# limanling/clip-event

Hardware: AMD Instinct MI355X
Metric: image-text pairs/sec/GPU, ViT-B/32 224px x 77-tok, global-batch contrastive (higher is better)
Workload: dtype bf16; 1 GPU; ViT-B/32 224px x 77-tok, bf16 operands, per-GPU batch 256, K=1, InfoNCE only, full train step (fwd+bwd+clip_grad_norm+Adam), random-init weights; global_batch=256, parallelism=dp1, captions=SOT + U[8,75] random ids + EOT, zero-padded to 77 (SURVEY 8(d) c2), text_rows=live tokens SOT..EOT only: 54.8% of B*77 rows (identical results, see DESIGN.md), fresh_captions_every_step=True, alignment=False, cu_hog=0, nt_pgrid=256, full=False

## Files before the change

clip_event_amd/csrc/attention.hip:

```cpp
#include <map>
#include <mutex>

#include <type_traits>

#include "common.hpp"
#include "../../include/clip_event_hip.h"

namespace {

constexpr int HD = 64;
constexpr int ROW = 160;

typedef __attribute__((address_space(3))) s16x4 lds_s16x4;
typedef __attribute__((ext_vector_type(8))) short s16x8;

__device__ __forceinline__ bf16x8 tr_pair(const char* p0, const char* p1) {
    s16x4 lo = __builtin_amdgcn_ds_read_tr16_b64_v4i16((lds_s16x4*)p0);
    s16x4 hi = __builtin_amdgcn_ds_read_tr16_b64_v4i16((lds_s16x4*)p1);
    s16x8 v = {lo[0], lo[1], lo[2], lo[3], hi[0], hi[1], hi[2], hi[3]};
    return __builtin_bit_cast(bf16x8, v);
}

__device__ __forceinline__ bf16x8 pack8(const f32x4& a, const f32x4& b) {
    u32x4 v = {pack_bf2(a[0], a[1]), pack_bf2(a[2], a[3]), pack_bf2(b[0], b[1]), pack_bf2(b[2], b[3])};
// ... 11 lines not shown
        const int idx = tid + j * nthr, r = idx >> 3, c = idx & 7;
        const uint32_t off = r < L ? (uint32_t)(r * ld * 2 + c * 16) : 0x80000000u;
        kv[j] = __builtin_amdgcn_raw_buffer_load_b128(rK, off, 0, 0);
        vv[j] = __builtin_amdgcn_raw_buffer_load_b128(rV, off, 0, 0);
    }
#pragma unroll
    for (int j = 0; j < NCH; ++j) {
        const int idx = tid + j * nthr, r = idx >> 3, c = idx & 7;
        if (idx < Lp * 8) {
            *reinterpret_cast<u32x4*>(sK + r * ROW + c * 16) = kv[j];
            *reinterpret_cast<u32x4*>(sV + r * ROW + c * 16) = vv[j];
        }
    }
}

template <int T>
__global__ __launch_bounds__(512) void attn_fwd_kernel(const bf16_t* __restrict__ qkv, long ld, bf16_t* __restrict__ o,
                                                       long ldo, float* __restrict__ lse,
                                                       const int* __restrict__ cu, int Lmax, int H, int D,
                                                       int causal, float scale) {
    extern __shared__ __attribute__((aligned(16))) char smem[];
    constexpr int Lp = T * 16;
    char* sK = smem;
    char* sV = smem + Lp * ROW;
    const int tid = threadIdx.x, lane = tid & 63;
    const int wave = __builtin_amdgcn_readfirstlane(tid >> 6), nw = blockDim.x >> 6;
    const int b = blockIdx.x / H, h = blockIdx.x - b * H;
    const long row0 = cu ? (long)cu[b] : (long)b * Lmax;
    const int L = cu ? min(cu[b + 1] - cu[b], Lmax) : Lmax;
    if (L <= 0) return;
    const int Tl = ((L + 31) >> 5) << 1;
    const bf16_t* base = qkv + row0 * ld + h * HD;

    const int li = lane & 15, g = lane >> 4;
    const int nstrips = (L + 15) >> 4;
    const int strip = wave;
    const int i = strip * 16 + li;
    const int iq = min(i, L - 1);
    bf16x8 qf[2];
    if (strip < nstrips) {
#pragma unroll
        for (int ks = 0; ks < 2; ++ks)
            qf[ks] = *reinterpret_cast<const bf16x8*>(base + (long)iq * ld + ks * 32 + g * 8);
    }
    stage_kv<4>(sK, sV, base + D, base + 2 * D, ld, L, Tl * 16, tid, blockDim.x);
    __syncthreads();

    if (strip < nstrips) {
        f32x4 s[T];
#pragma unroll
        for (int t = 0; t < T; ++t) {
            s[t] = f32x4{0.f, 0.f, 0.f, 0.f};
            if (t < Tl) {
#pragma unroll
                for (int ks = 0; ks < 2; ++ks) {
                    bf16x8 kf = *reinterpret_cast<const bf16x8*>(sK + (t * 16 + li) * ROW + (ks * 4 + g) * 16);
                    s[t] = __builtin_amdgcn_mfma_f32_16x16x32_bf16(kf, qf[ks], s[t], 0, 0, 0);
                }
            }
        }
        float mx = -INFINITY;
#pragma unroll
        for (int t = 0; t < T; ++t)
#pragma unroll
            for (int r = 0; r < 4; ++r) {
                const int j = t * 16 + g * 4 + r;
                const bool ok = (j < L) && (!causal || j <= i);
                s[t][r] = ok ? s[t][r] * scale : -INFINITY;
                mx = fmaxf(mx, s[t][r]);
            }
        mx = fmaxf(mx, __shfl_xor(mx, 16, 64));
        mx = fmaxf(mx, __shfl_xor(mx, 32, 64));
        float sum = 0.f;
#pragma unroll
        for (int t = 0; t < T; ++t)
#pragma unroll
            for (int r = 0; r < 4; ++r) {
                s[t][r] = __expf(s[t][r] - mx);
                sum += s[t][r];
            }
        sum += __shfl_xor(sum, 16, 64);
        sum += __shfl_xor(sum, 32, 64);
        f32x4 acc[4];
#pragma unroll
        for (int ct = 0; ct < 4; ++ct) acc[ct] = f32x4{0.f, 0.f, 0.f, 0.f};
#pragma unroll
        for (int sidx = 0; sidx < T / 2; ++sidx) {
            if (2 * sidx >= Tl) continue;
            bf16x8 pf = pack8(s[2 * sidx], s[2 * sidx + 1]);
            const char* vrow = sV + (32 * sidx + 4 * g + (li >> 2)) * ROW + (4 * (li & 3)) * 2;
#pragma unroll
            for (int ct = 0; ct < 4; ++ct) {
                bf16x8 vf = tr_pair(vrow + ct * 32, vrow + ct * 32 + 16 * ROW);
                acc[ct] = __builtin_amdgcn_mfma_f32_16x16x32_bf16(vf, pf, acc[ct], 0, 0, 0);
            }
        }
        if (i < L) {
            const float inv = 1.0f / sum;
            bf16_t* orow = o + (row0 + i) * ldo + h * HD + 4 * g;
#pragma unroll
            for (int ct = 0; ct < 4; ++ct) {
                u32x2 pk = {pack_bf2(acc[ct][0] * inv, acc[ct][1] * inv), pack_bf2(acc[ct][2] * inv, acc[ct][3] * inv)};
                *reinterpret_cast<u32x2*>(orow + ct * 16) = pk;
            }
            if (g == 0) lse[((long)b * H + h) * Lmax + i] = mx + __logf(sum);
        }
    }
}

template <int T>
__global__ __launch_bounds__(512) void attn_bwd_kernel(const bf16_t* __restrict__ qkv, long ld,
                                                       const bf16_t* __restrict__ o, long ldo,
                                                       const bf16_t* __restrict__ dout, long lddo,
                                                       const float* __restrict__ lse, bf16_t* __restrict__ dqkv,
                                                       long lddq, float* __restrict__ bias_grad,
                                                       const int* __restrict__ cu, int Lmax, int H, int D,
                                                       int causal, float scale) {
    extern __shared__ __attribute__((aligned(16))) char smem[];
    constexpr int Lp = T * 16;
    constexpr int PROW = Lp * 2 + 32;
    char* sA = smem;
    char* sB = sA + Lp * ROW;
    char* sP = sB + Lp * ROW;
    char* sDS = sP + Lp * PROW;
    auto csum = [&](int i) __attribute__((always_inline)) -> float* { return reinterpret_cast<float*>(sP + (i >> 3) * PROW + Lp * 2 + (i & 7) * 4); };
    const int tid = threadIdx.x, lane = tid & 63;
    const int wave = __builtin_amdgcn_readfirstlane(tid >> 6), nw = blockDim.x >> 6;
    const int b = blockIdx.x / H, h = blockIdx.x - b * H;
    const long row0 = cu ? (long)cu[b] : (long)b * Lmax;
    const int L = cu ? min(cu[b + 1] - cu[b], Lmax) : Lmax;
    if (L <= 0) return;
    const int Tl = ((L + 31) >> 5) << 1;
    const int Ll = Tl * 16;
    const bf16_t* base = qkv + row0 * ld + h * HD;
    const bf16_t* dob = dout + row0 * lddo + h * HD;
    const bf16_t* ob = o + row0 * ldo + h * HD;
    bf16_t* dbase = dqkv + row0 * lddq + h * HD;

    for (int i = tid; i < 192; i += blockDim.x) *csum(i) = 0.f;
    const int li = lane & 15, g = lane >> 4;
    u32x4 rK[2], rV[2], rQ[2], rD[2];
#pragma unroll
    for (int c = 0; c < 2; ++c) {
        const int idx = tid + c * blockDim.x;
        const int r = idx >> 3, ch = idx & 7;
        const u32x4 z = {0u, 0u, 0u, 0u};
        rK[c] = z; rV[c] = z; rQ[c] = z; rD[c] = z;
        if (idx < Ll * 8 && r < L) {
            rK[c] = *reinterpret_cast<const u32x4*>(base + D + (long)r * ld + ch * 8);
            rV[c] = *reinterpret_cast<const u32x4*>(base + 2 * D + (long)r * ld + ch * 8);
            rQ[c] = *reinterpret_cast<const u32x4*>(base + (long)r * ld + ch * 8);
            rD[c] = *reinterpret_cast<const u32x4*>(dob + (long)r * lddo + ch * 8);
        }
    }
    const int strip = wave;
    const bool has_strip = strip < Tl;
    const int i = strip * 16 + li;
    const bool iok = has_strip && i < L;
    const int iq = min(i, L - 1);
    float dl = 0.f, lsei = 0.f;
    bf16x8 qf[2], df[2];
    if (has_strip) {
        const u32x4* pd = reinterpret_cast<const u32x4*>(dob + (long)iq * lddo + g * 16);
        const u32x4* po = reinterpret_cast<const u32x4*>(ob + (long)iq * ldo + g * 16);
#pragma unroll
        for (int v = 0; v < 2; ++v) {
            u32x4 a = pd[v], c = po[v];
#pragma unroll
            for (int e = 0; e < 4; ++e) dl += bf_lo(a[e]) * bf_lo(c[e]) + bf_hi(a[e]) * bf_hi(c[e]);
        }
        lsei = lse[((long)b * H + h) * Lmax + iq];
#pragma unroll
        for (int ks = 0; ks < 2; ++ks) {
            qf[ks] = *reinterpret_cast<const bf16x8*>(base + (long)iq * ld + ks * 32 + g * 8);
            df[ks] = *reinterpret_cast<const bf16x8*>(dob + (long)iq * lddo + ks * 32 + g * 8);
        }
    }
#pragma unroll
    for (int c = 0; c < 2; ++c) {
        const int idx = tid + c * blockDim.x;
        if (idx < Ll * 8) {
            *reinterpret_cast<u32x4*>(sA + (idx >> 3) * ROW + (idx & 7) * 16) = rK[c];
            *reinterpret_cast<u32x4*>(sB + (idx >> 3) * ROW + (idx & 7) * 16) = rV[c];
        }
    }
    __syncthreads();
    dl += __shfl_xor(dl, 16, 64);
    dl += __shfl_xor(dl, 32, 64);

    if (has_strip) {
        f32x4 p[T], ds[T];
#pragma unroll
        for (int t = 0; t < T; ++t) {
            p[t] = f32x4{0.f, 0.f, 0.f, 0.f};
            ds[t] = f32x4{0.f, 0.f, 0.f, 0.f};
            if (t >= Tl) continue;
#pragma unroll
            for (int ks = 0; ks < 2; ++ks) {
                bf16x8 kf = *reinterpret_cast<const bf16x8*>(sA + (t * 16 + li) * ROW + (ks * 4 + g) * 16);
                bf16x8 vf = *reinterpret_cast<const bf16x8*>(sB + (t * 16 + li) * ROW + (ks * 4 + g) * 16);
                p[t] = __builtin_amdgcn_mfma_f32_16x16x32_bf16(kf, qf[ks], p[t], 0, 0, 0);
                ds[t] = __builtin_amdgcn_mfma_f32_16x16x32_bf16(vf, df[ks], ds[t], 0, 0, 0);
            }
#pragma unroll
            for (int r = 0; r < 4; ++r) {
                const int j = t * 16 + g * 4 + r;
                const bool ok = iok && (j < L) && (!causal || j <= i);
                const float pv = ok ? __expf(p[t][r] * scale - lsei) : 0.f;
                p[t][r] = pv;
                ds[t][r] = pv * (ds[t][r] - dl) * scale;
            }
            u32x2 pk = {pack_bf2(p[t][0], p[t][1]), pack_bf2(p[t][2], p[t][3])};
            u32x2 dk = {pack_bf2(ds[t][0], ds[t][1]), pack_bf2(ds[t][2], ds[t][3])};
            *reinterpret_cast<u32x2*>(sP + i * PROW + (t * 16 + g * 4) * 2) = pk;
            *reinterpret_cast<u32x2*>(sDS + i * PROW + (t * 16 + g * 4) * 2) = dk;
        }
        f32x4 acc[4];
#pragma unroll
        for (int ct = 0; ct < 4; ++ct) acc[ct] = f32x4{0.f, 0.f, 0.f, 0.f};
#pragma unroll
        for (int sidx = 0; sidx < T / 2; ++sidx) {
            if (2 * sidx >= Tl) continue;
            bf16x8 sf = pack8(ds[2 * sidx], ds[2 * sidx + 1]);
            const char* krow = sA + (32 * sidx + 4 * g + (li >> 2)) * ROW + (4 * (li & 3)) * 2;
#pragma unroll
            for (int ct = 0; ct < 4; ++ct) {
                bf16x8 kf = tr_pair(krow + ct * 32, krow + ct * 32 + 16 * ROW);
                acc[ct] = __builtin_amdgcn_mfma_f32_16x16x32_bf16(kf, sf, acc[ct], 0, 0, 0);
            }
        }
        if (iok) {
            bf16_t* qrow = dbase + (long)i * lddq + 4 * g;
#pragma unroll
            for (int ct = 0; ct < 4; ++ct) {
                u32x2 pk = {pack_bf2(acc[ct][0], acc[ct][1]), pack_bf2(acc[ct][2], acc[ct][3])};
                *reinterpret_cast<u32x2*>(qrow + ct * 16) = pk;
            }
// ... 19 lines not shown
        }
    }
    __syncthreads();
    const int nkt = (L + 15) >> 4;
    for (int jt = wave; jt < nkt; jt += nw) {
        const int j = jt * 16 + li;
        f32x4 av[4], ak[4];
#pragma unroll
        for (int ct = 0; ct < 4; ++ct) {
            av[ct] = f32x4{0.f, 0.f, 0.f, 0.f};
            ak[ct] = f32x4{0.f, 0.f, 0.f, 0.f};
        }
#pragma unroll
        for (int sidx = 0; sidx < T / 2; ++sidx) {
            if (2 * sidx >= Tl) continue;
            const int irow = 32 * sidx + 8 * g + (li >> 2);
            const char* pcol = sP + irow * PROW + (jt * 16 + 4 * (li & 3)) * 2;
            const char* scol = sDS + irow * PROW + (jt * 16 + 4 * (li & 3)) * 2;
            bf16x8 pf = tr_pair(pcol, pcol + 4 * PROW);
            bf16x8 sf = tr_pair(scol, scol + 4 * PROW);
            const int roff = irow * ROW + (4 * (li & 3)) * 2;
#pragma unroll
            for (int ct = 0; ct < 4; ++ct) {
                bf16x8 dof = tr_pair(sB + roff + ct * 32, sB + roff + ct * 32 + 4 * ROW);
                bf16x8 qf = tr_pair(sA + roff + ct * 32, sA + roff + ct * 32 + 4 * ROW);
                av[ct] = __builtin_amdgcn_mfma_f32_16x16x32_bf16(dof, pf, av[ct], 0, 0, 0);
                ak[ct] = __builtin_amdgcn_mfma_f32_16x16x32_bf16(qf, sf, ak[ct], 0, 0, 0);
            }
        }
        if (j < L) {
// ... 546 lines not shown
    }
    return e.p;
}

}

#define ATTN_DISPATCH(T, CALL)                 \
    switch (T) {                               \
        case 2: CALL(2); break;                \
        case 4: CALL(4); break;                \
        case 6: CALL(6); break;                \
        case 8: CALL(8); break;                \
        default: CE_CHECK_ARG(false, "attention: sequence length %d not supported", L); \
    }

extern "C" int ce_attention_fwd(const void* qkv, long ld, void* o, long ldo, float* lse, const int* cu_seqlens, int B,
                                int L, int H, int causal, void* stream) {
    CE_CHECK_ARG(B > 0 && L > 0 && H > 0, "ce_attention_fwd: empty problem");
    CE_CHECK_ARG(ld % 8 == 0 && ldo % 4 == 0, "ce_attention_fwd: ld must be a multiple of 8, ldo of 4");
    const int D = H * HD;
    if (L > 128) {
        CE_CHECK_ARG(!cu_seqlens, "ce_attention_fwd: packed batches are limited to 128 tokens per sample");
        CE_CHECK_ARG((long)B * H <= 65535, "ce_attention_fwd: B*H = %ld exceeds the grid", (long)B * H);
        hipStream_t sl = (hipStream_t)stream;
        CeProfScope prof(CE_PROF_ATTN_FWD, 4.0 * B * H * (double)L * L * HD, 2.0 * (double)B * L * (4.0 * D), sl);
        static const int ns = getenv("CE_ATTN_NS_FWD") ? atoi(getenv("CE_ATTN_NS_FWD")) : 1;
        if (ns == 1)
            hipLaunchKernelGGL(attn_fwd_long_kernel<1>, dim3((L + LB - 1) / LB, B * H), dim3(256), 0, sl, (const bf16_t*)qkv, ld,
                               (bf16_t*)o, ldo, lse, L, H, D, causal, 0.125f, attn_xcd_order());
        else
            hipLaunchKernelGGL(attn_fwd_long_kernel<2>, dim3((L + 2 * LB - 1) / (2 * LB), B * H), dim3(256), 0, sl, (const bf16_t*)qkv, ld,
                               (bf16_t*)o, ldo, lse, L, H, D, causal, 0.125f, attn_xcd_order());
        CE_LAUNCH_CHECK();
        return 0;
    }
    const int T = tiles_for(L);
    const int Lp = T * 16;
    int nw = (L + 15) / 16;
    if (nw > 8) nw = 8;
    const size_t lds = 2 * (size_t)Lp * ROW;
    const float scale = 0.125f;
    hipStream_t s = (hipStream_t)stream;
    CeProfScope prof(CE_PROF_ATTN_FWD, 4.0 * B * H * (double)L * L * HD, 2.0 * (double)B * L * (4.0 * D), s);
#define CALL(TT)                                                                                              \
    hipLaunchKernelGGL(attn_fwd_kernel<TT>, dim3(B * H), dim3(64 * nw), lds, s, (const bf16_t*)qkv, ld, (bf16_t*)o, ldo, \
                       lse, cu_seqlens, L, H, D, causal, scale)
    ATTN_DISPATCH(T, CALL);
#undef CALL
    CE_LAUNCH_CHECK();
    return 0;
}

extern "C" int ce_attention_bwd(const void* qkv, long ld, const void* o, long ldo, const void* dout, long lddo,
                                const float* lse, void* dqkv, long lddq, float* bias_grad, const int* cu_seqlens, int B,
                                int L, int H, int causal, void* stream) {
    CE_CHECK_ARG(B > 0 && L > 0 && H > 0, "ce_attention_bwd: empty problem");
    CE_CHECK_ARG(ld % 8 == 0 && ldo % 8 == 0 && lddo % 8 == 0 && lddq % 4 == 0, "ce_attention_bwd: bad leading dimension");
    const int D = H * HD;
    if (L > 128) {
        CE_CHECK_ARG(!cu_seqlens, "ce_attention_bwd: packed batches are limited to 128 tokens per sample");
        CE_CHECK_ARG((long)B * H <= 65535, "ce_attention_bwd: B*H = %ld exceeds the grid", (long)B * H);
        hipStream_t sl = (hipStream_t)stream;
        CeProfScope prof(CE_PROF_ATTN_BWD, 14.0 * B * H * (double)L * L * HD, 2.0 * (double)B * L * (8.0 * D), sl);
        static const int ns = getenv("CE_ATTN_NS") ? atoi(getenv("CE_ATTN_NS")) : 2;
        static const int nk = getenv("CE_ATTN_NK") ? atoi(getenv("CE_ATTN_NK")) : 1;
// ... 6 lines not shown
        if (ns == 1)
            hipLaunchKernelGGL(attn_bwd_long_dq_kernel<1>, grid1, dim3(256), 0, sl, (const bf16_t*)qkv, ld, (const bf16_t*)o, ldo,
                               (const bf16_t*)dout, lddo, lse, (bf16_t*)dqkv, lddq, bias_grad, delta, L, H, D, causal, 0.125f, attn_xcd_order());
        else
            hipLaunchKernelGGL(attn_bwd_long_dq_kernel<2>, grid2, dim3(256), 0, sl, (const bf16_t*)qkv, ld, (const bf16_t*)o, ldo,
                               (const bf16_t*)dout, lddo, lse, (bf16_t*)dqkv, lddq, bias_grad, delta, L, H, D, causal, 0.125f, attn_xcd_order());
        if (nk == 1)
            hipLaunchKernelGGL(attn_bwd_long_dkv_kernel<1>, grid1, dim3(256), 0, sl, (const bf16_t*)qkv, ld, (const bf16_t*)o, ldo,
                               (const bf16_t*)dout, lddo, lse, (bf16_t*)dqkv, lddq, bias_grad, delta, L, H, D, causal, 0.125f, attn_xcd_order());
        else
            hipLaunchKernelGGL(attn_bwd_long_dkv_kernel<2>, grid2, dim3(256), 0, sl, (const bf16_t*)qkv, ld, (const bf16_t*)o, ldo,
                               (const bf16_t*)dout, lddo, lse, (bf16_t*)dqkv, lddq, bias_grad, delta, L, H, D, causal, 0.125f, attn_xcd_order());
        CE_LAUNCH_CHECK();
        return 0;
    }
    const int T = tiles_for(L);
    const int Lp = T * 16;
    int nw = T;
    if (nw > 8) nw = 8;
    const size_t lds = 2 * (size_t)Lp * ROW + 2 * (size_t)Lp * (Lp * 2 + 32);
    const float scale = 0.125f;
    hipStream_t s = (hipStream_t)stream;
    CeProfScope prof(CE_PROF_ATTN_BWD, 10.0 * B * H * (double)L * L * HD, 2.0 * (double)B * L * (8.0 * D), s);
#define CALL(TT)                                                                                                   \
    do {                                                                                                           \
        static std::once_flag attr;                                                                                \
        std::call_once(attr, [] {                                                                                  \
            hipFuncSetAttribute(reinterpret_cast<const void*>(attn_bwd_kernel<TT>),                                \
                                hipFuncAttributeMaxDynamicSharedMemorySize, 160 * 1024);                           \
        });                                                                                                        \
        hipLaunchKernelGGL(attn_bwd_kernel<TT>, dim3(B * H), dim3(64 * nw), lds, s, (const bf16_t*)qkv, ld,        \
                           (const bf16_t*)o, ldo, (const bf16_t*)dout, lddo, lse, (bf16_t*)dqkv, lddq, bias_grad, cu_seqlens, L, \
                           H, D, causal, scale);                                                                           \
    } while (0)
    ATTN_DISPATCH(T, CALL);
#undef CALL
    CE_LAUNCH_CHECK();
    return 0;
}
```

clip_event_amd/csrc/tower.cpp:

```cpp
#include <hip/hip_runtime.h>
#include <stdlib.h>

#include <map>
#include <mutex>

#include "common.hpp"
#include "../../include/clip_event_hip.h"

namespace {

constexpr int WG_MAX_BLOCKS = 8;
constexpr int WG_SETS = WG_MAX_BLOCKS + 1;
constexpr int LNP_RING = 8;

struct Carver {
    char* base;
    size_t off = 0;
    explicit Carver(void* b) : base(reinterpret_cast<char*>(b)) {}
    template <typename T>
    T* take(size_t n) {
        off = (off + 255) & ~size_t(255);
        T* p = base ? reinterpret_cast<T*>(base + off) : nullptr;
        off += n * sizeof(T);
        return p;
// ... 113 lines not shown
        if (rc__ != 0) return rc__; \
    } while (0)

int linear(bool use8, const Layout& L, const void*& q8_of, const void* A, long lda, const void* W, const void* W8, const float* S8, int M,
           int N, int K, int epi, const float* bias, const void* resid, long ldr, void* out, long ldo, void* out2,
           long ldo2, const void* aux, long ldaux, void* stream) {
    if (use8 && W8 && S8 && K % 128 == 0 && K <= 4096) {
        if (q8_of != A || lda != K) TRY(ce_quant_rows_fp8(A, lda, L.q8, K, L.q8s, M, K, stream));
        q8_of = nullptr;
        return ce_gemm_nt_fp8(L.q8, K, L.q8s, W8, K, S8, M, N, K, epi, bias, resid, ldr, out, ldo, out2, ldo2, aux, ldaux,
                              stream);
    }
    return ce_gemm_nt(A, lda, W, K, M, N, K, epi, bias, resid, ldr, out, ldo, out2, ldo2, aux, ldaux, stream);
}

int forward_run(const ce_tower_desc* d, int batch, int rows, const int* cu_seqlens, const void* x0, Layout& L, void* x_out,
                const int* sel_rows, bool infer, void* stream) {
    const int M = rows, w = d->width;
    const bool f8 = (d->fp8 & 1) != 0;
    const int ST = d->stream16 ? CE_T_F16 : CE_T_F32;
    const int EPI_RESID = d->stream16 ? CE_EPI_BIAS_RESID_F16 : CE_EPI_BIAS_RESID_F32;
    const int EPI_FC = infer ? CE_EPI_BIAS_QGELU_BF16 : CE_EPI_BIAS_GELU;
    const long esz = d->stream16 ? 2 : 4;
    const void* x = x0;
    const void* q8_of = nullptr;
    const bool lnq = f8 && w % 128 == 0 && w <= 4096;
    for (int l = 0; l < d->layers; ++l) {
        const ce_block_params& p = d->blocks[l];
        BlockStash& s = L.blk[l];
        void* xo = (l + 1 < d->layers) ? s.x_out : x_out;
        TRY(ce_layernorm_fwd_q8(x, ST, w, nullptr, p.ln1_w, p.ln1_b, s.h1, CE_T_BF16, w, s.mean1, s.rstd1, M, w, 1e-5f,
                                lnq ? L.q8 : nullptr, w, L.q8s, stream));
        if (lnq) q8_of = s.h1;
        TRY(linear(f8, L, q8_of, s.h1, w, p.w_qkv, p.w8_qkv, p.s8_qkv, M, 3 * w, w, CE_EPI_BIAS_BF16, p.b_qkv, nullptr, 0, s.qkv, 3 * w, nullptr, 0,
                       nullptr, 0, stream));
        TRY(ce_attention_fwd(s.qkv, 3 * w, s.o, w, s.lse, cu_seqlens, batch, d->tokens, d->heads, d->causal, stream));
        if (sel_rows && l + 1 == d->layers) {
            const int Bn = batch;
            TRY(ce_copy_rows(s.o, w * 2L, sel_rows, L.os, w * 2L, nullptr, Bn, w * 2, stream));
            TRY(ce_copy_rows(x, w * esz, sel_rows, L.xs_in, w * esz, nullptr, Bn, (int)(w * esz), stream));
            TRY(linear(f8, L, q8_of, L.os, w, p.w_out, p.w8_out, p.s8_out, Bn, w, w, EPI_RESID, p.b_out, L.xs_in, w, L.xs_mid, w, nullptr,
                           0, nullptr, 0, stream));
            TRY(ce_layernorm_fwd_t(L.xs_mid, ST, w, nullptr, p.ln2_w, p.ln2_b, L.h2s, CE_T_BF16, w, L.means, L.rstds, Bn, w, 1e-5f, stream));
            TRY(linear(f8, L, q8_of, L.h2s, w, p.w_fc, p.w8_fc, p.s8_fc, Bn, 4 * w, w, EPI_FC, p.b_fc, nullptr, 0, infer ? L.gs : L.as, 4 * w,
                           infer ? nullptr : L.gs, infer ? 0 : 4 * w, nullptr, 0, stream));
            TRY(linear(f8, L, q8_of, L.gs, 4 * w, p.w_proj, p.w8_proj, p.s8_proj, Bn, w, 4 * w, EPI_RESID, p.b_proj, L.xs_mid, w, x_out, w,
                           nullptr, 0, nullptr, 0, stream));
            break;
        }
        TRY(linear(f8, L, q8_of, s.o, w, p.w_out, p.w8_out, p.s8_out, M, w, w, EPI_RESID, p.b_out, x, w, s.x_mid, w, nullptr, 0, nullptr,
                       0, stream));
        TRY(ce_layernorm_fwd_q8(s.x_mid, ST, w, nullptr, p.ln2_w, p.ln2_b, s.h2, CE_T_BF16, w, s.mean2, s.rstd2, M, w, 1e-5f,
                                lnq ? L.q8 : nullptr, w, L.q8s, stream));
        if (lnq) q8_of = s.h2;
// ... 140 lines not shown
        const int l = top, Bn = batch, q = l % WG_SETS;
        const ce_block_params& p = d->blocks[l];
        BlockStash& s = L.blk[l];
        const void* x_in = (l == 0) ? x0 : L.blk[l - 1].x_out;
        TRY(ce_cast_bf16(dx_sel, L.dxbs, (long)Bn * w, stream));
        TRY(linear(b8, L, q8_of, L.dxbs, w, p.wt_proj, p.wt8_proj, p.st8_proj, Bn, 4 * w, w, CE_EPI_GELUGRAD_BF16, nullptr, nullptr, 0, L.das, 4 * w, nullptr,
                       0, L.as, 4 * w, stream));
        TRY(ce_colsum_bf16(L.dxbs, w, p.g_b_proj, Bn, w, stream));
        TRY(linear(b8, L, q8_of, L.das, 4 * w, p.wt_fc, p.wt8_fc, p.st8_fc, Bn, w, 4 * w, CE_EPI_BF16, nullptr, nullptr, 0, L.dhs, w, nullptr, 0,
                       nullptr, 0, stream));
        TRY(ce_colsum_bf16(L.das, 4 * w, p.g_b_fc, Bn, 4 * w, stream));
        TRY(ce_layernorm_bwd_t(L.dhs, CE_T_BF16, w, L.xs_mid, ST, w, nullptr, L.means, L.rstds, p.ln2_w, dx_sel, CE_T_F32, L.dxs_mid,
                               ST, w, L.dxb2s, w, p.g_ln2_w, p.g_ln2_b, p.g_b_out, GS, Bn, w, stream));
        TRY(linear(b8, L, q8_of, L.dxb2s, w, p.wt_out, p.wt8_out, p.st8_out, Bn, w, w, CE_EPI_BF16, nullptr, nullptr, 0, L.dos, w, nullptr, 0, nullptr, 0,
                       stream));
        TRY(ce_scatter_rows_zero(L.dos, w * 2L, L.d_o, w * 2L, sel_rows, Bn, M, w * 2, stream));
        TRY(ce_attention_bwd(s.qkv, 3 * w, s.o, w, L.d_o, w, s.lse, L.dqkv[q], 3 * w, p.g_b_qkv, cu_seqlens, batch, d->tokens, d->heads,
                             d->causal, stream));
        {
            const void* P[3] = {L.dxbs, L.das, L.dxb2s};
            const long ldp[3] = {w, 4L * w, w};
            const void* Q[3] = {L.gs, L.h2s, L.os};
            const long ldq[3] = {4L * w, w, w};
            const int Nn[3] = {w, 4 * w, w};
            const int Kk[3] = {4 * w, w, w};
            float* out[3] = {p.g_w_proj, p.g_w_fc, p.g_w_out};
            const long ldo[3] = {4L * w, w, w};
            TRY(ce_gemm_tn_grouped_ex(3, P, ldp, Q, ldq, Bn, Nn, Kk, out, ldo, 0, d->wgrad_overwrite, stream));
        }
        queue(L.dqkv[q], 3L * w, s.h1, w, 3 * w, w, p.g_w_qkv, w);
        TRY(linear(b8, L, q8_of, L.dqkv[q], 3 * w, p.wt_qkv, p.wt8_qkv, p.st8_qkv, M, w, 3 * w, CE_EPI_BF16, nullptr, nullptr, 0, L.dh, w, nullptr, 0,
                       nullptr, 0, stream));
        TRY(ce_scatter_rows_zero(L.dxs_mid, w * esz, dx, w * esz, sel_rows, Bn, M, (int)(w * esz), stream));
// ... 45 lines not shown
```

clip_event_amd/ops.py:

```python
from __future__ import annotations

from ctypes import c_float, c_int, c_long, c_void_p
from typing import Optional

import torch

from . import _lib as L
from ._lib import check, lib, ptr, stream


def _rows(t: torch.Tensor) -> int:
    return t.shape[0]


def gemm_nt(a: torch.Tensor, b: torch.Tensor, epilogue: int, *, bias=None, resid=None, out=None, out2=None,
            aux=None, M: Optional[int] = None) -> torch.Tensor:
    assert a.dtype == torch.bfloat16 and b.dtype == torch.bfloat16 and a.is_cuda and b.is_cuda
    M = a.shape[0] if M is None else M
    K = a.shape[1]
    N = b.shape[0]
    assert b.shape[1] == K
    f32_out = epilogue in (L.EPI_F32, L.EPI_BIAS_F32, L.EPI_BIAS_RESID_F32)
    if epilogue == L.EPI_BIAS_RESID_F16:
        assert resid is not None and resid.dtype == torch.float16
# ... 89 lines not shown
    check(lib().ce_cast_t(ptr(x), c_int(_TYPE[x.dtype]), ptr(y), c_int(_TYPE[dtype]), c_float(mul), c_long(x.numel()), stream()),
          "ce_cast_t")
    return y


def attention_fwd(qkv: torch.Tensor, B: int, L: int, H: int, causal: bool, cu_seqlens=None):
    assert qkv.dtype == torch.bfloat16
    o = torch.empty(qkv.shape[0], H * 64, device=qkv.device, dtype=torch.bfloat16)
    lse = torch.empty(B * H * L, device=qkv.device, dtype=torch.float32)
    check(lib().ce_attention_fwd(ptr(qkv), c_long(qkv.stride(0)), ptr(o), c_long(o.stride(0)), ptr(lse),
                                 ptr(cu_seqlens), c_int(B), c_int(L), c_int(H), c_int(1 if causal else 0), stream()),
          "ce_attention_fwd")
    return o, lse


def attention_bwd(qkv, o, dout, lse, B: int, L: int, H: int, causal: bool, bias_grad=None, cu_seqlens=None):
    dqkv = torch.empty_like(qkv)
    check(lib().ce_attention_bwd(ptr(qkv), c_long(qkv.stride(0)), ptr(o), c_long(o.stride(0)), ptr(dout),
                                 c_long(dout.stride(0)), ptr(lse), ptr(dqkv), c_long(dqkv.stride(0)), ptr(bias_grad),
                                 ptr(cu_seqlens), c_int(B), c_int(L), c_int(H), c_int(1 if causal else 0), stream()),
          "ce_attention_bwd")
    return dqkv


def probe_mfma(shape: int, a_frags: torch.Tensor, b_frags: torch.Tensor) -> torch.Tensor:
    out = torch.empty(64, 4 if shape == 16 else 16, device=a_frags.device, dtype=torch.float32)
    check(lib().ce_probe_mfma(c_int(shape), ptr(a_frags), ptr(b_frags), ptr(out), stream()), "ce_probe_mfma")
    return out


def probe_tr16(image: torch.Tensor, byte_off: torch.Tensor) -> torch.Tensor:
    out = torch.empty(64, 4, device=image.device, dtype=torch.int16)
    check(lib().ce_probe_tr16(ptr(image), c_int(image.numel()), ptr(byte_off), ptr(out), stream()), "ce_probe_tr16")
    return out


# ... 70 lines not shown
```

include/clip_event_hip.h:

```cpp
#ifndef CLIP_EVENT_HIP_H
#define CLIP_EVENT_HIP_H

#include <stddef.h>
#include <stdint.h>

#ifdef __cplusplus
extern "C" {
#endif

const char* ce_last_error(void);
int ce_version(void);

enum {
    CE_EPI_BF16 = 0,
    CE_EPI_F32 = 1,
    CE_EPI_BIAS_BF16 = 2,
    CE_EPI_BIAS_F32 = 3,
    CE_EPI_BIAS_RESID_F32 = 4,
    CE_EPI_BIAS_GELU = 5,
    CE_EPI_GELUGRAD_BF16 = 6,
    CE_EPI_BIAS_RESID_F16 = 7,
    CE_EPI_BIAS_QGELU_BF16 = 8
};

// ... 64 lines not shown
                              const float* gscale, int M, int D, void* q8, long ldq, float* qscale, float* partials,
                              void* stream);
#define CE_LN_FOLD_MAX 64
typedef struct ce_ln_fold_job {
    const float* partials;
    float *dw, *db, *dxsum;
    int blocks, D;
} ce_ln_fold_job;
int ce_layernorm_fold(const ce_ln_fold_job* jobs , int njobs, void* stream);

int ce_attention_fwd(const void* qkv, long ld, void* o, long ldo, float* lse, const int* cu_seqlens, int B, int L,
                     int H, int causal, void* stream);
int ce_attention_bwd(const void* qkv, long ld, const void* o, long ldo, const void* dout, long lddo,
                     const float* lse, void* dqkv, long lddq, float* bias_grad, const int* cu_seqlens, int B, int L,
                     int H, int causal, void* stream);

int ce_im2col(const float* image, void* patches, int B, int resolution, int patch, int k_padded, void* stream);
int ce_vision_assemble(const float* patch_out, const float* cls, const float* pos, float* x0, int B, int tokens,
                       int D, void* stream);
int ce_vision_assemble_bwd(const float* dx0, void* dpatch, int B, int tokens, int D, void* stream);
int ce_token_embed(const int64_t* ids, const int* src_rows, const float* table, const float* pos, float* x0, long rows,
                   int tokens, int D, int vocab, void* stream);
int ce_token_embed_t(const int64_t* ids, const int* src_rows, const float* table, const float* pos, void* x0, int x0_type,
                     long rows, int tokens, int D, int vocab, void* stream);
int ce_token_embed_bwd(const int64_t* ids, const int* src_rows, const float* dx0, float* dtable, long rows, int D,
                       int vocab, void* stream);
int ce_pos_embed_bwd_packed(const float* dx0, const int* cu_seqlens, float* dpos, int n, int tokens, int D,
                            void* stream);
int ce_batch_reduce(const float* x, float* out, int B, long slab, long n, int accumulate, void* stream);
int ce_colsum_bf16(const void* x, long ld, float* out, int M, int N, void* stream);
// ... 173 lines not shown
```

Before: 20270 pairs/s (whole job).

## Add selected-row attention for last layer, causal tile skipping, and length-class launches

In the final transformer layer only the selected output row per sample (e.g. CLS/EOT) is needed. New fwd/bwd 'rows' kernels therefore compute attention only for that query strip, and the separate copy_rows and scatter_rows_zero passes are dropped. The kernels also gain compile-time causal and rows flags. With causal masking they skip key tiles above the diagonal using a per-strip unrolled dispatch. Packed variable-length batches are launched as several length classes so short sequences use smaller tile counts. This adds more template instantiations and launches, plus extra zeroing logic in the backward pass for strips that are not selected.

```diff
diff --git a/clip_event_amd/csrc/attention.hip b/clip_event_amd/csrc/attention.hip
--- a/clip_event_amd/csrc/attention.hip
+++ b/clip_event_amd/csrc/attention.hip
@@ -49,13 +49,27 @@
     }
 }
 
-template <int T>
+template <int N, class F>
+__device__ __forceinline__ void dispatch_upto(int v, F& f) {
+    if constexpr (N >= 1) {
+        if (v == N) f(std::integral_constant<int, N>{});
+        else dispatch_upto<N - 1>(v, f);
+    }
+}
+
+template <int T, bool CAUSAL, bool ROWS>
 __global__ __launch_bounds__(512) void attn_fwd_kernel(const bf16_t* __restrict__ qkv, long ld, bf16_t* __restrict__ o,
                                                        long ldo, float* __restrict__ lse,
-                                                       const int* __restrict__ cu, int Lmax, int H, int D,
-                                                       int causal, float scale) {
+                                                       const int* __restrict__ cu, const int* __restrict__ sel, int Lmax, int tl_min,
+                                                       int H, int D, float scale) {
     extern __shared__ __attribute__((aligned(16))) char smem[];
     constexpr int Lp = T * 16;
+    constexpr bool causal = CAUSAL;
+#ifdef CE_DIAG_NO_CAUSAL_SKIP
+    constexpr bool SKIP = false;
+#else
+    constexpr bool SKIP = CAUSAL;
+#endif
     char* sK = smem;
     char* sV = smem + Lp * ROW;
     const int tid = threadIdx.x, lane = tid & 63;
@@ -65,6 +79,7 @@
     const int L = cu ? min(cu[b + 1] - cu[b], Lmax) : Lmax;
     if (L <= 0) return;
     const int Tl = ((L + 31) >> 5) << 1;
+    if (Tl <= tl_min || Tl > T) return;
     const bf16_t* base = qkv + row0 * ld + h * HD;
 
     const int li = lane & 15, g = lane >> 4;
@@ -72,8 +87,14 @@
     const int strip = wave;
     const int i = strip * 16 + li;
     const int iq = min(i, L - 1);
+    int isel = 0;
+    if constexpr (ROWS) {
+        isel = (int)((long)sel[b] - row0);
+        if (isel < 0 || isel >= L) return;
+    }
+    const bool active = ROWS ? strip == (isel >> 4) : strip < nstrips;
     bf16x8 qf[2];
-    if (strip < nstrips) {
+    if (active) {
 #pragma unroll
         for (int ks = 0; ks < 2; ++ks)
             qf[ks] = *reinterpret_cast<const bf16x8*>(base + (long)iq * ld + ks * 32 + g * 8);
@@ -81,12 +102,14 @@
     stage_kv<4>(sK, sV, base + D, base + 2 * D, ld, L, Tl * 16, tid, blockDim.x);
     __syncthreads();
 
-    if (strip < nstrips) {
-        f32x4 s[T];
-#pragma unroll
-        for (int t = 0; t < T; ++t) {
+    auto strip_body = [&](auto te_tag) __attribute__((always_inline)) {
+        constexpr int TE = decltype(te_tag)::value;
+        constexpr int TP = TE + (TE & 1);
+        f32x4 s[TP];
+#pragma unroll
+        for (int t = 0; t < TP; ++t) {
             s[t] = f32x4{0.f, 0.f, 0.f, 0.f};
-            if (t < Tl) {
+            if (t < TE && (SKIP || t < Tl)) {
 #pragma unroll
                 for (int ks = 0; ks < 2; ++ks) {
                     bf16x8 kf = *reinterpret_cast<const bf16x8*>(sK + (t * 16 + li) * ROW + (ks * 4 + g) * 16);
@@ -96,7 +119,7 @@
         }
         float mx = -INFINITY;
 #pragma unroll
-        for (int t = 0; t < T; ++t)
+        for (int t = 0; t < TE; ++t)
 #pragma unroll
             for (int r = 0; r < 4; ++r) {
                 const int j = t * 16 + g * 4 + r;
@@ -108,7 +131,7 @@
         mx = fmaxf(mx, __shfl_xor(mx, 32, 64));
         float sum = 0.f;
 #pragma unroll
-        for (int t = 0; t < T; ++t)
+        for (int t = 0; t < TE; ++t)
 #pragma unroll
             for (int r = 0; r < 4; ++r) {
                 s[t][r] = __expf(s[t][r] - mx);
@@ -120,8 +143,8 @@
 #pragma unroll
         for (int ct = 0; ct < 4; ++ct) acc[ct] = f32x4{0.f, 0.f, 0.f, 0.f};
 #pragma unroll
-        for (int sidx = 0; sidx < T / 2; ++sidx) {
-            if (2 * sidx >= Tl) continue;
+        for (int sidx = 0; sidx < (TE + 1) / 2; ++sidx) {
+            if (!SKIP && 2 * sidx >= Tl) continue;
             bf16x8 pf = pack8(s[2 * sidx], s[2 * sidx + 1]);
             const char* vrow = sV + (32 * sidx + 4 * g + (li >> 2)) * ROW + (4 * (li & 3)) * 2;
 #pragma unroll
@@ -130,9 +153,9 @@
                 acc[ct] = __builtin_amdgcn_mfma_f32_16x16x32_bf16(vf, pf, acc[ct], 0, 0, 0);
             }
         }
-        if (i < L) {
+        if (ROWS ? i == isel : i < L) {
             const float inv = 1.0f / sum;
-            bf16_t* orow = o + (row0 + i) * ldo + h * HD + 4 * g;
+            bf16_t* orow = o + (ROWS ? (long)b : row0 + i) * ldo + h * HD + 4 * g;
 #pragma unroll
             for (int ct = 0; ct < 4; ++ct) {
                 u32x2 pk = {pack_bf2(acc[ct][0] * inv, acc[ct][1] * inv), pack_bf2(acc[ct][2] * inv, acc[ct][3] * inv)};
@@ -140,19 +163,29 @@
             }
             if (g == 0) lse[((long)b * H + h) * Lmax + i] = mx + __logf(sum);
         }
-    }
-}
-
-template <int T>
+    };
+    if (active) {
+        if constexpr (SKIP) dispatch_upto<T>(strip + 1, strip_body);
+        else strip_body(std::integral_constant<int, T>{});
+    }
+}
+
+template <int T, bool CAUSAL, bool ROWS>
 __global__ __launch_bounds__(512) void attn_bwd_kernel(const bf16_t* __restrict__ qkv, long ld,
                                                        const bf16_t* __restrict__ o, long ldo,
                                                        const bf16_t* __restrict__ dout, long lddo,
                                                        const float* __restrict__ lse, bf16_t* __restrict__ dqkv,
                                                        long lddq, float* __restrict__ bias_grad,
-                                                       const int* __restrict__ cu, int Lmax, int H, int D,
-                                                       int causal, float scale) {
+                                                       const int* __restrict__ cu, const int* __restrict__ sel, int Lmax, int tl_min,
+                                                       int H, int D, float scale) {
     extern __shared__ __attribute__((aligned(16))) char smem[];
     constexpr int Lp = T * 16;
+    constexpr bool causal = CAUSAL;
+#ifdef CE_DIAG_NO_CAUSAL_SKIP
+    constexpr bool SKIP = false;
+#else
+    constexpr bool SKIP = CAUSAL;
+#endif
     constexpr int PROW = Lp * 2 + 32;
     char* sA = smem;
     char* sB = sA + Lp * ROW;
@@ -166,11 +199,18 @@
     const int L = cu ? min(cu[b + 1] - cu[b], Lmax) : Lmax;
     if (L <= 0) return;
     const int Tl = ((L + 31) >> 5) << 1;
+    if (Tl <= tl_min || Tl > T) return;
     const int Ll = Tl * 16;
     const bf16_t* base = qkv + row0 * ld + h * HD;
-    const bf16_t* dob = dout + row0 * lddo + h * HD;
-    const bf16_t* ob = o + row0 * ldo + h * HD;
+    const bf16_t* dob = dout + (ROWS ? (long)b : row0) * lddo + h * HD;
+    const bf16_t* ob = o + (ROWS ? (long)b : row0) * ldo + h * HD;
     bf16_t* dbase = dqkv + row0 * lddq + h * HD;
+    int isel = -1;
+    if constexpr (ROWS) {
+        isel = (int)((long)sel[b] - row0);
+        if (isel < 0 || isel >= L) isel = -1;
+    }
+    const int ssel = isel >> 4;
 
     for (int i = tid; i < 192; i += blockDim.x) *csum(i) = 0.f;
     const int li = lane & 15, g = lane >> 4;
@@ -185,30 +225,40 @@
             rK[c] = *reinterpret_cast<const u32x4*>(base + D + (long)r * ld + ch * 8);
             rV[c] = *reinterpret_cast<const u32x4*>(base + 2 * D + (long)r * ld + ch * 8);
             rQ[c] = *reinterpret_cast<const u32x4*>(base + (long)r * ld + ch * 8);
-            rD[c] = *reinterpret_cast<const u32x4*>(dob + (long)r * lddo + ch * 8);
+            if constexpr (ROWS) {
+                if (r == isel) rD[c] = *reinterpret_cast<const u32x4*>(dob + ch * 8);
+            } else {
+                rD[c] = *reinterpret_cast<const u32x4*>(dob + (long)r * lddo + ch * 8);
+            }
         }
     }
     const int strip = wave;
     const bool has_strip = strip < Tl;
+    const bool mine = ROWS ? strip == ssel : has_strip;
     const int i = strip * 16 + li;
     const bool iok = has_strip && i < L;
+    const bool qok = ROWS ? i == isel : iok;
     const int iq = min(i, L - 1);
     float dl = 0.f, lsei = 0.f;
     bf16x8 qf[2], df[2];
-    if (has_strip) {
-        const u32x4* pd = reinterpret_cast<const u32x4*>(dob + (long)iq * lddo + g * 16);
-        const u32x4* po = reinterpret_cast<const u32x4*>(ob + (long)iq * ldo + g * 16);
-#pragma unroll
-        for (int v = 0; v < 2; ++v) {
-            u32x4 a = pd[v], c = po[v];
-#pragma unroll
-            for (int e = 0; e < 4; ++e) dl += bf_lo(a[e]) * bf_lo(c[e]) + bf_hi(a[e]) * bf_hi(c[e]);
-        }
-        lsei = lse[((long)b * H + h) * Lmax + iq];
+    if (mine) {
+        const long drow = ROWS ? 0 : (long)iq * lddo, orow = ROWS ? 0 : (long)iq * ldo;
+        if (!ROWS || qok) {
+            const u32x4* pd = reinterpret_cast<const u32x4*>(dob + drow + g * 16);
+            const u32x4* po = reinterpret_cast<const u32x4*>(ob + orow + g * 16);
+#pragma unroll
+            for (int v = 0; v < 2; ++v) {
+                u32x4 a = pd[v], c = po[v];
+#pragma unroll
+                for (int e = 0; e < 4; ++e) dl += bf_lo(a[e]) * bf_lo(c[e]) + bf_hi(a[e]) * bf_hi(c[e]);
+            }
+            lsei = lse[((long)b * H + h) * Lmax + iq];
+        }
 #pragma unroll
         for (int ks = 0; ks < 2; ++ks) {
             qf[ks] = *reinterpret_cast<const bf16x8*>(base + (long)iq * ld + ks * 32 + g * 8);
-            df[ks] = *reinterpret_cast<const bf16x8*>(dob + (long)iq * lddo + ks * 32 + g * 8);
+            if (!ROWS || qok) df[ks] = *reinterpret_cast<const bf16x8*>(dob + drow + ks * 32 + g * 8);
+            else df[ks] = __builtin_bit_cast(bf16x8, u32x4{0u, 0u, 0u, 0u});
         }
     }
 #pragma unroll
@@ -223,13 +273,38 @@
     dl += __shfl_xor(dl, 16, 64);
     dl += __shfl_xor(dl, 32, 64);
 
-    if (has_strip) {
+    if (ROWS && has_strip && !mine) {
+        const u32x2 z = {0u, 0u};
+        if (iok) {
+            bf16_t* qrow = dbase + (long)i * lddq + 4 * g;
+#pragma unroll
+            for (int ct = 0; ct < 4; ++ct) *reinterpret_cast<u32x2*>(qrow + ct * 16) = z;
+        }
+        if (strip == (ssel ^ 1)) {
+#pragma unroll
+            for (int t = 0; t < T; ++t) {
+                if (t >= Tl) continue;
+                *reinterpret_cast<u32x2*>(sP + i * PROW + (t * 16 + g * 4) * 2) = z;
+                *reinterpret_cast<u32x2*>(sDS + i * PROW + (t * 16 + g * 4) * 2) = z;
+            }
+        }
+    }
+    if (mine) {
+        const int tend = SKIP ? min(Tl, strip + 1) : Tl;
         f32x4 p[T], ds[T];
 #pragma unroll
         for (int t = 0; t < T; ++t) {
             p[t] = f32x4{0.f, 0.f, 0.f, 0.f};
             ds[t] = f32x4{0.f, 0.f, 0.f, 0.f};
             if (t >= Tl) continue;
+            if (SKIP && t >= tend) {
+                if (t == (strip | 1)) {
+                    const u32x2 z = {0u, 0u};
+                    *reinterpret_cast<u32x2*>(sP + i * PROW + (t * 16 + g * 4) * 2) = z;
+                    *reinterpret_cast<u32x2*>(sDS + i * PROW + (t * 16 + g * 4) * 2) = z;
+                }
+                continue;
+            }
 #pragma unroll
             for (int ks = 0; ks < 2; ++ks) {
                 bf16x8 kf = *reinterpret_cast<const bf16x8*>(sA + (t * 16 + li) * ROW + (ks * 4 + g) * 16);
@@ -240,7 +315,7 @@
 #pragma unroll
             for (int r = 0; r < 4; ++r) {
                 const int j = t * 16 + g * 4 + r;
-                const bool ok = iok && (j < L) && (!causal || j <= i);
+                const bool ok = qok && (j < L) && (!causal || j <= i);
                 const float pv = ok ? __expf(p[t][r] * scale - lsei) : 0.f;
                 p[t][r] = pv;
                 ds[t][r] = pv * (ds[t][r] - dl) * scale;
@@ -255,7 +330,7 @@
         for (int ct = 0; ct < 4; ++ct) acc[ct] = f32x4{0.f, 0.f, 0.f, 0.f};
 #pragma unroll
         for (int sidx = 0; sidx < T / 2; ++sidx) {
-            if (2 * sidx >= Tl) continue;
+            if (2 * sidx >= tend) continue;
             bf16x8 sf = pack8(ds[2 * sidx], ds[2 * sidx + 1]);
             const char* krow = sA + (32 * sidx + 4 * g + (li >> 2)) * ROW + (4 * (li & 3)) * 2;
 #pragma unroll
@@ -305,6 +380,8 @@
 #pragma unroll
         for (int sidx = 0; sidx < T / 2; ++sidx) {
             if (2 * sidx >= Tl) continue;
+            if (ROWS && sidx != (ssel >> 1)) continue;
+            if (SKIP && 2 * sidx + 1 < jt) continue;
             const int irow = 32 * sidx + 8 * g + (li >> 2);
             const char* pcol = sP + irow * PROW + (jt * 16 + 4 * (li & 3)) * 2;
             const char* scol = sDS + irow * PROW + (jt * 16 + 4 * (li & 3)) * 2;
@@ -881,6 +958,87 @@
         default: CE_CHECK_ARG(false, "attention: sequence length %d not supported", L); \
     }
 
+namespace {
+
+struct LengthClasses { int n, T[4], lo[4]; };
+LengthClasses length_classes(int L, bool packed) {
+    LengthClasses c{};
+    const int top = tiles_for(L);
+#ifdef CE_DIAG_ONE_CLASS
+    packed = false;
+#endif
+    if (!packed) { c.n = 1; c.T[0] = top; c.lo[0] = 0; return c; }
+#ifdef CE_ATTN_TWO_CLASSES
+    if (top > 4) { c.n = 2; c.T[0] = 4; c.lo[0] = 0; c.T[1] = top; c.lo[1] = 4; }
+    else { c.n = 1; c.T[0] = top; c.lo[0] = 0; }
+#else
+    for (int t = 2; t <= top; t += 2) { c.T[c.n] = t; c.lo[c.n] = t - 2; ++c.n; }
+#endif
+    return c;
+}
+
+template <bool ROWS>
+int attention_fwd_short(const void* qkv, long ld, void* o, long ldo, float* lse, const int* cu_seqlens, const int* sel, int B, int L,
+                        int H, int causal, hipStream_t s) {
+    const int D = H * HD;
+    const float scale = 0.125f;
+    const LengthClasses cls = length_classes(L, cu_seqlens != nullptr);
+    for (int k = 0; k < cls.n; ++k) {
+        const int T = cls.T[k], lo = cls.lo[k];
+        int nw = (k + 1 == cls.n) ? (L + 15) / 16 : T;
+        if (nw > 8) nw = 8;
+        const size_t lds = 2 * (size_t)T * 16 * ROW;
+#define CALL(TT)                                                                                                               \
+    do {                                                                                                                       \
+        if (causal)                                                                                                            \
+            hipLaunchKernelGGL((attn_fwd_kernel<TT, true, ROWS>), dim3(B * H), dim3(64 * nw), lds, s, (const bf16_t*)qkv, ld,  \
+                               (bf16_t*)o, ldo, lse, cu_seqlens, sel, L, lo, H, D, scale);                                     \
+        else                                                                                                                   \
+            hipLaunchKernelGGL((attn_fwd_kernel<TT, false, ROWS>), dim3(B * H), dim3(64 * nw), lds, s, (const bf16_t*)qkv, ld, \
+                               (bf16_t*)o, ldo, lse, cu_seqlens, sel, L, lo, H, D, scale);                                     \
+    } while (0)
+        ATTN_DISPATCH(T, CALL);
+#undef CALL
+    }
+    CE_LAUNCH_CHECK();
+    return 0;
+}
+
+template <int T, bool CAUSAL, bool ROWS>
+void launch_bwd_short(const void* qkv, long ld, const void* o, long ldo, const void* dout, long lddo, const float* lse, void* dqkv,
+                      long lddq, float* bias_grad, const int* cu_seqlens, const int* sel, int B, int L, int lo, int H, hipStream_t s) {
+    static std::once_flag attr;
+    std::call_once(attr, [] {
+        hipFuncSetAttribute(reinterpret_cast<const void*>(attn_bwd_kernel<T, CAUSAL, ROWS>), hipFuncAttributeMaxDynamicSharedMemorySize,
+                            160 * 1024);
+    });
+    constexpr int Lp = T * 16;
+    const size_t lds = 2 * (size_t)Lp * ROW + 2 * (size_t)Lp * (Lp * 2 + 32);
+    hipLaunchKernelGGL((attn_bwd_kernel<T, CAUSAL, ROWS>), dim3(B * H), dim3(64 * T), lds, s, (const bf16_t*)qkv, ld, (const bf16_t*)o,
+                       ldo, (const bf16_t*)dout, lddo, lse, (bf16_t*)dqkv, lddq, bias_grad, cu_seqlens, sel, L, lo, H, H * HD, 0.125f);
+}
+
+template <bool ROWS>
+int attention_bwd_short(const void* qkv, long ld, const void* o, long ldo, const void* dout, long lddo, const float* lse, void* dqkv,
+                        long lddq, float* bias_grad, const int* cu_seqlens, const int* sel, int B, int L, int H, int causal,
+                        hipStream_t s) {
+    const LengthClasses cls = length_classes(L, cu_seqlens != nullptr);
+    for (int k = 0; k < cls.n; ++k) {
+        const int T = cls.T[k], lo = cls.lo[k];
+#define CALL(TT)                                                                                                                     \
+    do {                                                                                                                             \
+        if (causal) launch_bwd_short<TT, true, ROWS>(qkv, ld, o, ldo, dout, lddo, lse, dqkv, lddq, bias_grad, cu_seqlens, sel, B, L, lo, H, s);  \
+        else launch_bwd_short<TT, false, ROWS>(qkv, ld, o, ldo, dout, lddo, lse, dqkv, lddq, bias_grad, cu_seqlens, sel, B, L, lo, H, s);        \
+    } while (0)
+        ATTN_DISPATCH(T, CALL);
+#undef CALL
+    }
+    CE_LAUNCH_CHECK();
+    return 0;
+}
+
+}
+
 extern "C" int ce_attention_fwd(const void* qkv, long ld, void* o, long ldo, float* lse, const int* cu_seqlens, int B,
                                 int L, int H, int causal, void* stream) {
     CE_CHECK_ARG(B > 0 && L > 0 && H > 0, "ce_attention_fwd: empty problem");
@@ -901,21 +1059,19 @@
         CE_LAUNCH_CHECK();
         return 0;
     }
-    const int T = tiles_for(L);
-    const int Lp = T * 16;
-    int nw = (L + 15) / 16;
-    if (nw > 8) nw = 8;
-    const size_t lds = 2 * (size_t)Lp * ROW;
-    const float scale = 0.125f;
     hipStream_t s = (hipStream_t)stream;
     CeProfScope prof(CE_PROF_ATTN_FWD, 4.0 * B * H * (double)L * L * HD, 2.0 * (double)B * L * (4.0 * D), s);
-#define CALL(TT)                                                                                              \
-    hipLaunchKernelGGL(attn_fwd_kernel<TT>, dim3(B * H), dim3(64 * nw), lds, s, (const bf16_t*)qkv, ld, (bf16_t*)o, ldo, \
-                       lse, cu_seqlens, L, H, D, causal, scale)
-    ATTN_DISPATCH(T, CALL);
-#undef CALL
-    CE_LAUNCH_CHECK();
-    return 0;
+    return attention_fwd_short<false>(qkv, ld, o, ldo, lse, cu_seqlens, nullptr, B, L, H, causal, s);
+}
+
+extern "C" int ce_attention_fwd_rows(const void* qkv, long ld, void* o_sel, long ldo, float* lse, const int* cu_seqlens,
+                                     const int* sel_rows, int B, int L, int H, int causal, void* stream) {
+    CE_CHECK_ARG(B > 0 && L > 0 && H > 0, "ce_attention_fwd_rows: empty problem");
+    CE_CHECK_ARG(L <= 128, "ce_attention_fwd_rows: at most 128 tokens per sample (got %d)", L);
+    CE_CHECK_ARG(sel_rows && ld % 8 == 0 && ldo % 4 == 0, "ce_attention_fwd_rows: sel_rows missing, or ld not a multiple of 8 / ldo of 4");
+    hipStream_t s = (hipStream_t)stream;
+    CeProfScope prof(CE_PROF_ATTN_FWD, 4.0 * B * H * 16.0 * L * HD, 2.0 * (double)B * L * (2.0 * H * HD), s);
+    return attention_fwd_short<true>(qkv, ld, o_sel, ldo, lse, cu_seqlens, sel_rows, B, L, H, causal, s);
 }
 
 extern "C" int ce_attention_bwd(const void* qkv, long ld, const void* o, long ldo, const void* dout, long lddo,
@@ -952,27 +1108,20 @@
         CE_LAUNCH_CHECK();
         return 0;
     }
-    const int T = tiles_for(L);
-    const int Lp = T * 16;
-    int nw = T;
-    if (nw > 8) nw = 8;
-    const size_t lds = 2 * (size_t)Lp * ROW + 2 * (size_t)Lp * (Lp * 2 + 32);
-    const float scale = 0.125f;
     hipStream_t s = (hipStream_t)stream;
     CeProfScope prof(CE_PROF_ATTN_BWD, 10.0 * B * H * (double)L * L * HD, 2.0 * (double)B * L * (8.0 * D), s);
-#define CALL(TT)                                                                                                   \
-    do {                                                                                                           \
-        static std::once_flag attr;                                                                                \
-        std::call_once(attr, [] {                                                                                  \
-            hipFuncSetAttribute(reinterpret_cast<const void*>(attn_bwd_kernel<TT>),                                \
-                                hipFuncAttributeMaxDynamicSharedMemorySize, 160 * 1024);                           \
-        });                                                                                                        \
-        hipLaunchKernelGGL(attn_bwd_kernel<TT>, dim3(B * H), dim3(64 * nw), lds, s, (const bf16_t*)qkv, ld,        \
-                           (const bf16_t*)o, ldo, (const bf16_t*)dout, lddo, lse, (bf16_t*)dqkv, lddq, bias_grad, cu_seqlens, L, \
-                           H, D, causal, scale);                                                                           \
-    } while (0)
-    ATTN_DISPATCH(T, CALL);
-#undef CALL
-    CE_LAUNCH_CHECK();
-    return 0;
-}
+    return attention_bwd_short<false>(qkv, ld, o, ldo, dout, lddo, lse, dqkv, lddq, bias_grad, cu_seqlens, nullptr, B, L, H, causal, s);
+}
+
+extern "C" int ce_attention_bwd_rows(const void* qkv, long ld, const void* o_sel, long ldo, const void* dout_sel, long lddo,
+                                     const float* lse, void* dqkv, long lddq, float* bias_grad, const int* cu_seqlens,
+                                     const int* sel_rows, int B, int L, int H, int causal, void* stream) {
+    CE_CHECK_ARG(B > 0 && L > 0 && H > 0, "ce_attention_bwd_rows: empty problem");
+    CE_CHECK_ARG(L <= 128, "ce_attention_bwd_rows: at most 128 tokens per sample (got %d)", L);
+    CE_CHECK_ARG(sel_rows && ld % 8 == 0 && ldo % 8 == 0 && lddo % 8 == 0 && lddq % 4 == 0,
+                 "ce_attention_bwd_rows: sel_rows missing, or a bad leading dimension");
+    hipStream_t s = (hipStream_t)stream;
+    CeProfScope prof(CE_PROF_ATTN_BWD, 10.0 * B * H * 32.0 * L * HD, 2.0 * (double)B * L * (6.0 * H * HD), s);
+    return attention_bwd_short<true>(qkv, ld, o_sel, ldo, dout_sel, lddo, lse, dqkv, lddq, bias_grad, cu_seqlens, sel_rows, B, L, H,
+                                     causal, s);
+}
diff --git a/clip_event_amd/csrc/tower.cpp b/clip_event_amd/csrc/tower.cpp
--- a/clip_event_amd/csrc/tower.cpp
+++ b/clip_event_amd/csrc/tower.cpp
@@ -151,6 +151,11 @@
     return ce_gemm_nt(A, lda, W, K, M, N, K, epi, bias, resid, ldr, out, ldo, out2, ldo2, aux, ldaux, stream);
 }
 
+#ifdef CE_DIAG_NO_ROWS
+constexpr bool ROWS_ATTN = false;
+#else
+constexpr bool ROWS_ATTN = true;
+#endif
 int forward_run(const ce_tower_desc* d, int batch, int rows, const int* cu_seqlens, const void* x0, Layout& L, void* x_out,
                 const int* sel_rows, bool infer, void* stream) {
     const int M = rows, w = d->width;
@@ -171,10 +176,14 @@
         if (lnq) q8_of = s.h1;
         TRY(linear(f8, L, q8_of, s.h1, w, p.w_qkv, p.w8_qkv, p.s8_qkv, M, 3 * w, w, CE_EPI_BIAS_BF16, p.b_qkv, nullptr, 0, s.qkv, 3 * w, nullptr, 0,
                        nullptr, 0, stream));
-        TRY(ce_attention_fwd(s.qkv, 3 * w, s.o, w, s.lse, cu_seqlens, batch, d->tokens, d->heads, d->causal, stream));
-        if (sel_rows && l + 1 == d->layers) {
+        const bool pruned = sel_rows && l + 1 == d->layers;
+        if (pruned && ROWS_ATTN && d->tokens <= 128)
+            TRY(ce_attention_fwd_rows(s.qkv, 3 * w, L.os, w, s.lse, cu_seqlens, sel_rows, batch, d->tokens, d->heads, d->causal, stream));
+        else
+            TRY(ce_attention_fwd(s.qkv, 3 * w, s.o, w, s.lse, cu_seqlens, batch, d->tokens, d->heads, d->causal, stream));
+        if (pruned) {
             const int Bn = batch;
-            TRY(ce_copy_rows(s.o, w * 2L, sel_rows, L.os, w * 2L, nullptr, Bn, w * 2, stream));
+            if (!(ROWS_ATTN && d->tokens <= 128)) TRY(ce_copy_rows(s.o, w * 2L, sel_rows, L.os, w * 2L, nullptr, Bn, w * 2, stream));
             TRY(ce_copy_rows(x, w * esz, sel_rows, L.xs_in, w * esz, nullptr, Bn, (int)(w * esz), stream));
             TRY(linear(f8, L, q8_of, L.os, w, p.w_out, p.w8_out, p.s8_out, Bn, w, w, EPI_RESID, p.b_out, L.xs_in, w, L.xs_mid, w, nullptr,
                            0, nullptr, 0, stream));
@@ -345,9 +354,14 @@
                                ST, w, L.dxb2s, w, p.g_ln2_w, p.g_ln2_b, p.g_b_out, GS, Bn, w, stream));
         TRY(linear(b8, L, q8_of, L.dxb2s, w, p.wt_out, p.wt8_out, p.st8_out, Bn, w, w, CE_EPI_BF16, nullptr, nullptr, 0, L.dos, w, nullptr, 0, nullptr, 0,
                        stream));
-        TRY(ce_scatter_rows_zero(L.dos, w * 2L, L.d_o, w * 2L, sel_rows, Bn, M, w * 2, stream));
-        TRY(ce_attention_bwd(s.qkv, 3 * w, s.o, w, L.d_o, w, s.lse, L.dqkv[q], 3 * w, p.g_b_qkv, cu_seqlens, batch, d->tokens, d->heads,
-                             d->causal, stream));
+        if (ROWS_ATTN && d->tokens <= 128) {
+            TRY(ce_attention_bwd_rows(s.qkv, 3 * w, L.os, w, L.dos, w, s.lse, L.dqkv[q], 3 * w, p.g_b_qkv, cu_seqlens, sel_rows, batch,
+                                      d->tokens, d->heads, d->causal, stream));
+        } else {
+            TRY(ce_scatter_rows_zero(L.dos, w * 2L, L.d_o, w * 2L, sel_rows, Bn, M, w * 2, stream));
+            TRY(ce_attention_bwd(s.qkv, 3 * w, s.o, w, L.d_o, w, s.lse, L.dqkv[q], 3 * w, p.g_b_qkv, cu_seqlens, batch, d->tokens, d->heads,
+                                 d->causal, stream));
+        }
         {
             const void* P[3] = {L.dxbs, L.das, L.dxb2s};
             const long ldp[3] = {w, 4L * w, w};
diff --git a/clip_event_amd/ops.py b/clip_event_amd/ops.py
--- a/clip_event_amd/ops.py
+++ b/clip_event_amd/ops.py
@@ -127,12 +127,36 @@
     return o, lse
 
 
-def attention_bwd(qkv, o, dout, lse, B: int, L: int, H: int, causal: bool, bias_grad=None, cu_seqlens=None):
-    dqkv = torch.empty_like(qkv)
+def attention_bwd(qkv, o, dout, lse, B: int, L: int, H: int, causal: bool, bias_grad=None, cu_seqlens=None, dqkv=None):
+    if dqkv is None:
+        dqkv = torch.empty_like(qkv)
     check(lib().ce_attention_bwd(ptr(qkv), c_long(qkv.stride(0)), ptr(o), c_long(o.stride(0)), ptr(dout),
                                  c_long(dout.stride(0)), ptr(lse), ptr(dqkv), c_long(dqkv.stride(0)), ptr(bias_grad),
                                  ptr(cu_seqlens), c_int(B), c_int(L), c_int(H), c_int(1 if causal else 0), stream()),
           "ce_attention_bwd")
+    return dqkv
+
+
+def attention_fwd_rows(qkv, sel_rows, B: int, L: int, H: int, causal: bool, cu_seqlens=None, lse=None):
+    assert qkv.dtype == torch.bfloat16 and sel_rows.dtype == torch.int32
+    o = torch.empty(B, H * 64, device=qkv.device, dtype=torch.bfloat16)
+    if lse is None:
+        lse = torch.empty(B * H * L, device=qkv.device, dtype=torch.float32)
+    check(lib().ce_attention_fwd_rows(ptr(qkv), c_long(qkv.stride(0)), ptr(o), c_long(o.stride(0)), ptr(lse), ptr(cu_seqlens),
+                                      ptr(sel_rows), c_int(B), c_int(L), c_int(H), c_int(1 if causal else 0), stream()),
+          "ce_attention_fwd_rows")
+    return o, lse
+
+
+def attention_bwd_rows(qkv, o_sel, dout_sel, lse, sel_rows, B: int, L: int, H: int, causal: bool, bias_grad=None, cu_seqlens=None,
+                       dqkv=None):
+    assert sel_rows.dtype == torch.int32
+    if dqkv is None:
+        dqkv = torch.empty_like(qkv)
+    check(lib().ce_attention_bwd_rows(ptr(qkv), c_long(qkv.stride(0)), ptr(o_sel), c_long(o_sel.stride(0)), ptr(dout_sel),
+                                      c_long(dout_sel.stride(0)), ptr(lse), ptr(dqkv), c_long(dqkv.stride(0)), ptr(bias_grad),
+                                      ptr(cu_seqlens), ptr(sel_rows), c_int(B), c_int(L), c_int(H), c_int(1 if causal else 0),
+                                      stream()), "ce_attention_bwd_rows")
     return dqkv
 
 
diff --git a/include/clip_event_hip.h b/include/clip_event_hip.h
--- a/include/clip_event_hip.h
+++ b/include/clip_event_hip.h
@@ -102,6 +102,12 @@
 int ce_attention_bwd(const void* qkv, long ld, const void* o, long ldo, const void* dout, long lddo,
                      const float* lse, void* dqkv, long lddq, float* bias_grad, const int* cu_seqlens, int B, int L,
                      int H, int causal, void* stream);
+
+int ce_attention_fwd_rows(const void* qkv, long ld, void* o_sel, long ldo, float* lse, const int* cu_seqlens, const int* sel_rows,
+                          int B, int L, int H, int causal, void* stream);
+int ce_attention_bwd_rows(const void* qkv, long ld, const void* o_sel, long ldo, const void* dout_sel, long lddo, const float* lse,
+                          void* dqkv, long lddq, float* bias_grad, const int* cu_seqlens, const int* sel_rows, int B, int L, int H,
+                          int causal, void* stream);
 
 int ce_im2col(const float* image, void* patches, int B, int resolution, int patch, int k_padded, void* stream);
 int ce_vision_assemble(const float* patch_out, const float* cls, const float* pos, float* x0, int B, int tokens,
```

Result: slower. 19760 pairs/s (whole job) (-2.5%).
